# KaffinPX/neptune-core

Measured on AMD Instinct MI355X. Metric: STARK proofs verified/sec (whole node) + Tip5 perms/sec vs VALU roofline, higher is better.
Workload: dtype u64 (Goldilocks mod p; XFE = cubic extension)

## Files before the change

neptune-core_amd/csrc/stark_kernels.hip:

```cpp
#include <hip/hip_ext.h>

#include <atomic>
#include <cstdlib>
#include <type_traits>

#include "../../include/nhip_challenge_id.h"
#include "kernels.hpp"
#include "proof_codec.hpp"
#include "stark.hpp"
#include "stark_launch_plan.hpp"
#include "tip5_device.hpp"
#include "xfe.hpp"

namespace nhip {

#ifndef NHIP_LAT_PRIO
#define NHIP_LAT_PRIO 2
#endif
__device__ __forceinline__ void latency_priority() {
    if constexpr (NHIP_LAT_PRIO > 0) __builtin_amdgcn_s_setprio(NHIP_LAT_PRIO);
}
__device__ uint32_t g_batches_done;
struct AgePrio {
    uint32_t seq, k;
// ... 219 lines not shown
                s[1] = 4 + e < rem ? word_mont<MW>(c1) : (4 + e == rem ? MONT_ONE : 0ull);
                if (r2) s[2] = 8 + e < rem ? word_mont<MW>(c2) : (8 + e == rem ? MONT_ONE : 0ull);
                tip5_permute_quad(s, cq, rck, e, lds.lut);
            }
        } else if (op.kind == FS_SQUEEZE_X) {
            const uint32_t nwords = 3 * op.n;
            for (uint32_t f = 0; f < nwords; f += TIP5_RATE) {
                if (f + e < nwords) xs[xcur + f + e] = s[0];
                if (f + 4 + e < nwords) xs[xcur + f + 4 + e] = s[1];
                if (r2 && f + 8 + e < nwords) xs[xcur + f + 8 + e] = s[2];
                tip5_permute_quad(s, cq, rck, e, lds.lut);
            }
            xcur += nwords;
        } else {
            const uint64_t bound = op.arg;
            uint32_t got = 0;
            while (got < op.n) {
                const uint64_t v0 = from_mont(s[0]), v1 = from_mont(s[1]), v2 = from_mont(s[2]);
                tip5_permute_quad(s, cq, rck, e, lds.lut);
                const bool ok0 = v0 != GL_P - 1, ok1 = v1 != GL_P - 1, ok2 = r2 && v2 != GL_P - 1;
                const uint64_t b0 = __ballot(ok0), b1 = __ballot(ok1), b2 = __ballot(ok2);
                const uint32_t bits = ((uint32_t)(b0 >> qb) & 0xFu) | (((uint32_t)(b1 >> qb) & 0xFu) << 4) |
                                      (((uint32_t)(b2 >> qb) & 0x3u) << 8);
                auto put = [&](bool ok, uint32_t w, uint64_t v) {
                    const uint32_t rank = __popc(bits & ((1u << w) - 1u));
                    if (ok && got + rank < op.n) idx_out[icur + got + rank] = (uint32_t)((v & 0xFFFFFFFFull) % bound);
                };
                put(ok0, e, v0);
                put(ok1, 4 + e, v1);
                put(ok2, 8 + e, v2);
                got += __popc(bits);
            }
            icur += op.n;
        }
    }
}

#ifndef NHIP_ROWS_WAVES
#define NHIP_ROWS_WAVES 5
#endif
#ifndef NHIP_ROWS_WAVES_PLANES
#define NHIP_ROWS_WAVES_PLANES 4
#endif
template <bool MW, bool PLANES>
__global__ void __launch_bounds__(256, PLANES ? NHIP_ROWS_WAVES_PLANES : NHIP_ROWS_WAVES) k_hash_rows(const uint64_t* __restrict__ words, const ProofDesc* __restrict__ desc,
                                                   uint32_t n_proofs, uint32_t k, StarkDims dims,
                                                   uint64_t* __restrict__ dig, const uint32_t* __restrict__ fail,
                                                   AgePrio age) {
    age_priority(age, 0);
    __shared__ Tip5Lds lds;
    tip5_lds_init(lds);
    std::conditional_t<PLANES, Tip5Planes, Tip5NoPlanes> pl;
    if constexpr (PLANES) tip5_planes_init(pl);
    const uint32_t tree = blockIdx.y;
    const uint32_t width = tree == 0 ? dims.num_main : (tree == 1 ? 3 * dims.num_aux : 3 * dims.num_quot_seg);
    for (uint64_t t = blockIdx.x * (uint64_t)blockDim.x + threadIdx.x; t < (uint64_t)n_proofs * k;
         t += (uint64_t)gridDim.x * blockDim.x) {
        const uint32_t p = (uint32_t)(t / k), j = (uint32_t)(t % k);
        if (fail[p]) continue;
        const ProofDesc& d = desc[p];
        const uint64_t base = (tree == 0 ? d.main_rows_off : (tree == 1 ? d.aux_rows_off : d.quot_rows_off)) +
                              (uint64_t)j * width;
        const uint64_t* __restrict__ row = words + base;
        uint64_t s[16];
#pragma unroll
        for (int q = 0; q < 16; ++q) s[q] = 0;
        const uint32_t nchunks = width / TIP5_RATE + 1;
        for (uint32_t c = 0; c < nchunks; ++c) {
            const uint32_t pos = c * TIP5_RATE;
            const bool last = c + 1 == nchunks;
            if (!last) {
#pragma unroll
                for (int q = 0; q < TIP5_RATE; ++q) s[q] = word_mont<MW>(row[pos + q]);
            } else {
                const uint32_t rem = width - pos;
#pragma unroll
                for (int q = 0; q < TIP5_RATE; ++q) {
                    const uint32_t qq = (uint32_t)q;
                    s[q] = qq < rem ? word_mont<MW>(row[pos + qq]) : (qq == rem ? MONT_ONE : 0ull);
                }
            }
            tip5_rounds_0_3(s, lds.lut, pl);
            tip5_last_sbox(s, lds.lut);
            if (!last) tip5_last_mds<10, 16>(s);
            else tip5_last_mds<0, 5>(s);
        }
        uint64_t* __restrict__ o = dig + (((uint64_t)p * 3 + tree) * k + j) * 5;
#pragma unroll
        for (int q = 0; q < 5; ++q) o[q] = s[q];
    }
}

template <bool MW>
__device__ __forceinline__ void hash_rows_wide_body(uint32_t bx, uint32_t tree, const Tip5Lds& t5,
                                                    const uint64_t* __restrict__ words,
                                                    const ProofDesc* __restrict__ desc, uint32_t n_proofs,
                                                    uint32_t k, StarkDims dims, uint64_t* __restrict__ dig,
                                                    const uint32_t* __restrict__ fail) {
    const uint32_t width = tree == 0 ? dims.num_main : (tree == 1 ? 3 * dims.num_aux : 3 * dims.num_quot_seg);
    const uint32_t e = threadIdx.x & 15u;
    const uint64_t t = ((uint64_t)bx * blockDim.x + threadIdx.x) >> 4;
    if (t >= (uint64_t)n_proofs * k) return;
    const uint32_t p = (uint32_t)(t / k), j = (uint32_t)(t % k);
    if (fail[p]) return;
    const ProofDesc& d = desc[p];
    const uint64_t* __restrict__ row =
        words + (tree == 0 ? d.main_rows_off : (tree == 1 ? d.aux_rows_off : d.quot_rows_off)) + (uint64_t)j * width;
    uint64_t rcs[TIP5_ROUNDS];
#pragma unroll
    for (int r = 0; r < TIP5_ROUNDS; ++r) rcs[r] = c_tip5_rc_raw[r * 16 + e];
    const uint32_t nchunks = width / TIP5_RATE + 1;
    auto chunk_word = [&](uint32_t c) -> uint64_t {
        const uint32_t pos = c * TIP5_RATE;
        if (c + 1 < nchunks) return e < TIP5_RATE ? word_mont<MW>(row[pos + e]) : 0ull;
        const uint32_t rem = width - pos;
        return e < rem ? word_mont<MW>(row[pos + e]) : (e == rem ? MONT_ONE : 0ull);
    };
    uint64_t s = 0, next = chunk_word(0);
    for (uint32_t c = 0; c < nchunks; ++c) {
        if (e < TIP5_RATE) s = next;
        if (c + 1 < nchunks) next = chunk_word(c + 1);
        s = tip5_permute_wide<true>(s, e, rcs, t5.lut);
    }
    if (e < 5) dig[(((uint64_t)p * 3 + tree) * k + j) * 5 + e] = s;
}
template <bool MW>
__global__ void __launch_bounds__(256) k_hash_rows_wide(const uint64_t* __restrict__ words,
                                                        const ProofDesc* __restrict__ desc, uint32_t n_proofs,
                                                        uint32_t k, StarkDims dims, uint64_t* __restrict__ dig,
                                                        const uint32_t* __restrict__ fail) {
    latency_priority();
    __shared__ Tip5Lds t5;
    tip5_lds_init(t5);
    hash_rows_wide_body<MW>(blockIdx.x, blockIdx.y, t5, words, desc, n_proofs, k, dims, dig, fail);
}

template <bool MW>
__global__ void __launch_bounds__(256) k_fs_rows_small(const uint64_t* __restrict__ words,
                                                       const ProofDesc* __restrict__ desc,
                                                       const FsOp* __restrict__ ops, uint32_t n_proofs,
                                                       uint64_t* __restrict__ xs, uint32_t* __restrict__ idx_out,
                                                       const uint32_t* __restrict__ fail, AgePrio age,
                                                       uint32_t fs_blocks, uint32_t rows_gx, uint32_t k,
                                                       StarkDims dims, uint64_t* __restrict__ dig) {
    const uint32_t bx = blockIdx.x;
    if (bx < fs_blocks) age_priority(age, NHIP_LAT_PRIO);
    else latency_priority();
    __shared__ Tip5Lds lds;
    tip5_lds_init(lds);
    if (bx < fs_blocks) {
        fs_replay_wide_body<true, MW>(bx, lds, words, desc, ops, n_proofs, xs, idx_out, fail);
    } else {
        const uint32_t r = bx - fs_blocks;
        hash_rows_wide_body<MW>(r % rows_gx, r / rows_gx, lds, words, desc, n_proofs, k, dims, dig, fail);
    }
}

__device__ __forceinline__ void hash_pair_raw(const uint64_t* l, const uint64_t* r, uint64_t* out,
                                              const uint8_t* __restrict__ lut) {
    uint64_t s[16];
#pragma unroll
    for (int q = 0; q < 5; ++q) {
        s[q] = l[q];
        s[5 + q] = r[q];
    }
    tip5_hash_pair_digest(s, lut);
#pragma unroll
// ... 1354 lines not shown
```

neptune-core_amd/csrc/tip5_device.hpp:

```cpp
#pragma once
#include "goldilocks.hpp"
#include "tip5_constants.h"
#include "tip5_mds_planes.hpp"

namespace nhip {

static constexpr int TIP5_STATE = 16;
static constexpr int TIP5_RATE = 10;
static constexpr int TIP5_ROUNDS = 5;
static constexpr uint64_t MONT_ONE = 0x00000000FFFFFFFFull;

__constant__ static uint64_t c_tip5_rc_raw[80] = {
#define NHIP_RC(i) TIP5_RC_RAW[i]
    NHIP_RC(0), NHIP_RC(1), NHIP_RC(2), NHIP_RC(3), NHIP_RC(4), NHIP_RC(5), NHIP_RC(6), NHIP_RC(7),
    NHIP_RC(8), NHIP_RC(9), NHIP_RC(10), NHIP_RC(11), NHIP_RC(12), NHIP_RC(13), NHIP_RC(14), NHIP_RC(15),
    NHIP_RC(16), NHIP_RC(17), NHIP_RC(18), NHIP_RC(19), NHIP_RC(20), NHIP_RC(21), NHIP_RC(22), NHIP_RC(23),
    NHIP_RC(24), NHIP_RC(25), NHIP_RC(26), NHIP_RC(27), NHIP_RC(28), NHIP_RC(29), NHIP_RC(30), NHIP_RC(31),
    NHIP_RC(32), NHIP_RC(33), NHIP_RC(34), NHIP_RC(35), NHIP_RC(36), NHIP_RC(37), NHIP_RC(38), NHIP_RC(39),
    NHIP_RC(40), NHIP_RC(41), NHIP_RC(42), NHIP_RC(43), NHIP_RC(44), NHIP_RC(45), NHIP_RC(46), NHIP_RC(47),
    NHIP_RC(48), NHIP_RC(49), NHIP_RC(50), NHIP_RC(51), NHIP_RC(52), NHIP_RC(53), NHIP_RC(54), NHIP_RC(55),
    NHIP_RC(56), NHIP_RC(57), NHIP_RC(58), NHIP_RC(59), NHIP_RC(60), NHIP_RC(61), NHIP_RC(62), NHIP_RC(63),
    NHIP_RC(64), NHIP_RC(65), NHIP_RC(66), NHIP_RC(67), NHIP_RC(68), NHIP_RC(69), NHIP_RC(70), NHIP_RC(71),
    NHIP_RC(72), NHIP_RC(73), NHIP_RC(74), NHIP_RC(75), NHIP_RC(76), NHIP_RC(77), NHIP_RC(78), NHIP_RC(79),
#undef NHIP_RC
};

__constant__ static uint64_t c_tip5_rck_raw[80] = {
#define NHIP_RC(i) (TIP5_RC_RAW[i] + 0xFFFFFFFFull)
    NHIP_RC(0), NHIP_RC(1), NHIP_RC(2), NHIP_RC(3), NHIP_RC(4), NHIP_RC(5), NHIP_RC(6), NHIP_RC(7),
    NHIP_RC(8), NHIP_RC(9), NHIP_RC(10), NHIP_RC(11), NHIP_RC(12), NHIP_RC(13), NHIP_RC(14), NHIP_RC(15),
    NHIP_RC(16), NHIP_RC(17), NHIP_RC(18), NHIP_RC(19), NHIP_RC(20), NHIP_RC(21), NHIP_RC(22), NHIP_RC(23),
    NHIP_RC(24), NHIP_RC(25), NHIP_RC(26), NHIP_RC(27), NHIP_RC(28), NHIP_RC(29), NHIP_RC(30), NHIP_RC(31),
    NHIP_RC(32), NHIP_RC(33), NHIP_RC(34), NHIP_RC(35), NHIP_RC(36), NHIP_RC(37), NHIP_RC(38), NHIP_RC(39),
    NHIP_RC(40), NHIP_RC(41), NHIP_RC(42), NHIP_RC(43), NHIP_RC(44), NHIP_RC(45), NHIP_RC(46), NHIP_RC(47),
    NHIP_RC(48), NHIP_RC(49), NHIP_RC(50), NHIP_RC(51), NHIP_RC(52), NHIP_RC(53), NHIP_RC(54), NHIP_RC(55),
    NHIP_RC(56), NHIP_RC(57), NHIP_RC(58), NHIP_RC(59), NHIP_RC(60), NHIP_RC(61), NHIP_RC(62), NHIP_RC(63),
    NHIP_RC(64), NHIP_RC(65), NHIP_RC(66), NHIP_RC(67), NHIP_RC(68), NHIP_RC(69), NHIP_RC(70), NHIP_RC(71),
    NHIP_RC(72), NHIP_RC(73), NHIP_RC(74), NHIP_RC(75), NHIP_RC(76), NHIP_RC(77), NHIP_RC(78), NHIP_RC(79),
#undef NHIP_RC
};

struct Tip5Lds {
    uint8_t lut[256];
};

__host__ __device__ constexpr uint32_t tip5_lut_entry(uint32_t x) {
    return ((((x + 1u) * (x + 1u)) % 257u * (x + 1u)) % 257u + 256u) % 257u;
}
constexpr bool tip5_lut_formula_matches_table() {
    for (uint32_t x = 0; x < 256; ++x)
        if (tip5_lut_entry(x) != TIP5_LUT[x]) return false;
    return true;
}
static_assert(tip5_lut_formula_matches_table(), "L(x) = (x+1)^3 - 1 mod 257 is the Tip5 lookup table");

__device__ __forceinline__ void tip5_lds_init(Tip5Lds& lds) {
    for (int i = threadIdx.x; i < 256; i += blockDim.x) lds.lut[i] = TIP5_LUT[i];
    __syncthreads();
}

__device__ __forceinline__ uint32_t lookup4(const uint8_t* __restrict__ lut, uint32_t w) {
    const uint32_t b0 = lut[w & 0xFFu];
    const uint32_t b1 = lut[(w >> 8) & 0xFFu];
    const uint32_t b2 = lut[(w >> 16) & 0xFFu];
    const uint32_t b3 = lut[w >> 24];
    return b0 | (b1 << 8) | (b2 << 16) | (b3 << 24);
}

__device__ __forceinline__ uint64_t split_and_lookup(const uint8_t* __restrict__ lut, uint64_t r) {
    const uint32_t lo = lookup4(lut, (uint32_t)r);
    const uint32_t hi = lookup4(lut, (uint32_t)(r >> 32));
    return ((uint64_t)hi << 32) | lo;
}

__device__ __forceinline__ uint64_t pow7(uint64_t x) {
    const uint64_t x2 = mont_sqr(x);
    const uint64_t x4 = mont_sqr(x2);
    const uint64_t x3 = mont_mul(x, x2);
    return mont_mul(x3, x4);
}

#ifndef NHIP_POW7_GROUP
#define NHIP_POW7_GROUP 3
#endif
__device__ __forceinline__ void mad_carry3(const uint32_t* a1, const uint32_t* b0, const uint64_t* t, uint64_t* u,
                                           uint32_t* c) {
    uint64_t g0, g1, g2;
    asm("v_mad_u64_u32 %0, %6, %9, %12, %15\n\t"
        "v_mad_u64_u32 %1, %7, %10, %13, %16\n\t"
        "v_mad_u64_u32 %2, %8, %11, %14, %17\n\t"
        "v_cndmask_b32_e64 %3, 0, 1, %6\n\t"
        "v_cndmask_b32_e64 %4, 0, 1, %7\n\t"
        "v_cndmask_b32_e64 %5, 0, 1, %8"
        : "=&v"(u[0]), "=&v"(u[1]), "=&v"(u[2]), "=v"(c[0]), "=v"(c[1]), "=v"(c[2]), "=&s"(g0), "=&s"(g1),
          "=&s"(g2)
        : "v"(a1[0]), "v"(a1[1]), "v"(a1[2]), "v"(b0[0]), "v"(b0[1]), "v"(b0[2]), "v"(t[0]), "v"(t[1]), "v"(t[2]));
}

template <int N>
__device__ __forceinline__ void mont_mul_n_dev(const uint64_t* a, const uint64_t* b, uint64_t* out) {
    static_assert(N % 3 == 0, "groups of three");
    uint64_t p00[N], t[N], u[N], xh[N];
    uint32_t a1[N], b0[N], c[N];
    uint32_t ah[N], e[N], bl[N], bh[N], rl[N], rh[N], c1[N], cc[N];
#pragma unroll
    for (int i = 0; i < N; ++i) {
        a1[i] = (uint32_t)(a[i] >> 32);
        b0[i] = (uint32_t)b[i];
        p00[i] = (uint64_t)(uint32_t)a[i] * b0[i];
    }
#pragma unroll
    for (int i = 0; i < N; ++i) t[i] = (uint64_t)(uint32_t)a[i] * (uint32_t)(b[i] >> 32) + (p00[i] >> 32);
#pragma unroll
    for (int i = 0; i < N; i += 3) mad_carry3(a1 + i, b0 + i, t + i, u + i, c + i);
#pragma unroll
    for (int i = 0; i < N; ++i)
        xh[i] = (uint64_t)a1[i] * (uint32_t)(b[i] >> 32) + (((uint64_t)c[i] << 32) | (uint32_t)(u[i] >> 32));
#pragma unroll
    for (int i = 0; i < N; ++i) ah[i] = __builtin_addc((uint32_t)u[i], (uint32_t)p00[i], 0u, &e[i]);
#pragma unroll
    for (int i = 0; i < N; ++i) {
        unsigned int br1;
        bl[i] = __builtin_subc((uint32_t)p00[i], ah[i], e[i], &br1);
        e[i] = br1;
    }
#pragma unroll
    for (int i = 0; i < N; ++i) {
        unsigned int br2;
        bh[i] = __builtin_subc(ah[i], 0u, e[i], &br2);
    }
#pragma unroll
    for (int i = 0; i < N; ++i) rl[i] = __builtin_subc((uint32_t)xh[i], bl[i], 0u, &c1[i]);
#pragma unroll
    for (int i = 0; i < N; ++i) rh[i] = __builtin_subc((uint32_t)(xh[i] >> 32), bh[i], c1[i], &cc[i]);
#pragma unroll
    for (int i = 0; i < N; ++i) {
        unsigned int c2;
        const uint32_t lo = __builtin_subc(rl[i], 0u - cc[i], 0u, &c2);
        out[i] = ((uint64_t)(rh[i] - c2) << 32) | lo;
    }
}

template <int G>
__device__ __forceinline__ void pow7_mul(const uint64_t* a, const uint64_t* b, uint64_t* out) {
    mont_mul_n_dev<G>(a, b, out);
}

__device__ __forceinline__ void pow7_12(uint64_t* x) {
    constexpr int G = NHIP_POW7_GROUP;
    static_assert(12 % G == 0, "group must divide 12");
#pragma unroll
    for (int g = 0; g < 12; g += G) {
        uint64_t x2[G], x4[G], x3[G];
        pow7_mul<G>(x + g, x + g, x2);
        pow7_mul<G>(x2, x2, x4);
        pow7_mul<G>(x + g, x2, x3);
        pow7_mul<G>(x3, x4, x + g);
    }
}

__device__ __forceinline__ void mds_fold4(const uint32_t* sh, const uint64_t* slo, uint64_t* w, uint32_t* e) {
    uint64_t g0, g1, g2, g3;
    asm("v_mad_u64_u32 %0, %8, %12, -1, %16\n\t"
        "v_mad_u64_u32 %1, %9, %13, -1, %17\n\t"
        "v_mad_u64_u32 %2, %10, %14, -1, %18\n\t"
        "v_mad_u64_u32 %3, %11, %15, -1, %19\n\t"
        "v_cndmask_b32_e64 %4, -1, 0, %8\n\t"
        "v_cndmask_b32_e64 %5, -1, 0, %9\n\t"
        "v_cndmask_b32_e64 %6, -1, 0, %10\n\t"
        "v_cndmask_b32_e64 %7, -1, 0, %11"
        : "=&v"(w[0]), "=&v"(w[1]), "=&v"(w[2]), "=&v"(w[3]), "=v"(e[0]), "=v"(e[1]), "=v"(e[2]), "=v"(e[3]),
          "=&s"(g0), "=&s"(g1), "=&s"(g2), "=&s"(g3)
        : "v"(sh[0]), "v"(sh[1]), "v"(sh[2]), "v"(sh[3]), "v"(slo[0]), "v"(slo[1]), "v"(slo[2]), "v"(slo[3]));
}

__device__ __forceinline__ uint64_t mds_reduce_fold(uint64_t al, uint64_t ah);
template <int NIN, int I0, int N>
__device__ __forceinline__ void mds_fold_outputs(const uint32_t* lo, const uint32_t* hi,
                                                 const uint64_t* __restrict__ rck, uint64_t* out) {
    uint64_t al[N], ah[N];
#pragma unroll
    for (int o = 0; o < N; ++o) {
        const int i = I0 + o;
        al[o] = rck[i];
        ah[o] = 0;
#pragma unroll
        for (int j = 0; j < NIN; ++j) {
            const uint64_t c = TIP5_MDS[(i - j) & 15];
            al[o] += c * lo[j];
            ah[o] += c * hi[j];
        }
    }
    constexpr int N4 = N & ~3;
    uint32_t sh[N4 > 0 ? N4 : 1];
    uint64_t slo[N4 > 0 ? N4 : 1], w[N4 > 0 ? N4 : 1];
    uint32_t e[N4 > 0 ? N4 : 1];
#pragma unroll
    for (int o = 0; o < N4; ++o) {
        unsigned int k;
        const uint32_t m1 = __builtin_addc((uint32_t)(al[o] >> 32), (uint32_t)ah[o], 0u, &k);
        sh[o] = (uint32_t)(ah[o] >> 32) + k;
        slo[o] = ((uint64_t)m1 << 32) | (uint32_t)al[o];
    }
#pragma unroll
    for (int o = 0; o < N4; o += 4) mds_fold4(sh + o, slo + o, w + o, e + o);
#pragma unroll
    for (int o = 0; o < N4; ++o) out[o] = w[o] - e[o];
#pragma unroll
    for (int o = N4; o < N; ++o) out[o] = mds_reduce_fold(al[o], ah[o]);
}

#ifndef NHIP_PAIR_MDS_GROUP
#define NHIP_PAIR_MDS_GROUP 2
#endif
#ifndef NHIP_SPONGE_MDS_GROUP
#define NHIP_SPONGE_MDS_GROUP 4
#endif
template <int NIN, int OBEG, int OEND, int G>
__device__ __forceinline__ void mds_fold_groups(const uint32_t* lo, const uint32_t* hi,
                                                const uint64_t* __restrict__ rck, uint64_t* out) {
    constexpr int N = (OEND - OBEG) < G ? (OEND - OBEG) : G;
    mds_fold_outputs<NIN, OBEG, N>(lo, hi, rck, out);
    if constexpr (OBEG + N < OEND) {
        __builtin_amdgcn_sched_barrier(0);
        mds_fold_groups<NIN, OBEG + N, OEND, G>(lo, hi, rck, out + N);
    }
}

template <int NIN, int OBEG = 0, int OEND = 16, int G = 16>
__device__ __forceinline__ void mds_ark_fold(uint64_t s[16], const uint64_t* __restrict__ rck) {
    uint32_t lo[NIN], hi[NIN];
#pragma unroll
    for (int j = 0; j < NIN; ++j) {
        lo[j] = (uint32_t)s[j];
        hi[j] = (uint32_t)(s[j] >> 32);
    }
    uint64_t out[OEND - OBEG];
    mds_fold_groups<NIN, OBEG, OEND, G>(lo, hi, rck, out);
#pragma unroll
    for (int o = 0; o < OEND - OBEG; ++o) s[OBEG + o] = out[o];
}

template <int G = NHIP_SPONGE_MDS_GROUP>
__device__ __forceinline__ void mds_ark(uint64_t s[16], const uint64_t* __restrict__ rc,
                                        const uint64_t* __restrict__ rck) {
    (void)rc;
    mds_ark_fold<16, 0, 16, G>(s, rck);
}

typedef int tip5_v4i __attribute__((ext_vector_type(4)));
typedef int tip5_v16i __attribute__((ext_vector_type(16)));

struct Tip5PlanesTable {
    uint32_t w[3 * 64 * 4];
};
constexpr Tip5PlanesTable tip5_planes_table() {
    Tip5PlanesTable tb{};
    for (int e = 0; e < 3; ++e)
        for (int l = 0; l < 64; ++l)
            for (int t = 0; t < 16; ++t)
                tb.w[(e * 64 + l) * 4 + t / 4] |= (uint32_t)(uint8_t)(int8_t)planes_tile_byte(e, l, t) << (8 * (t % 4));
    return tb;
}
__constant__ static Tip5PlanesTable c_tip5_planes_tiles = tip5_planes_table();

__constant__ static uint64_t c_tip5_rckp_raw[80] = {
#define NHIP_RC(i) planes_start(TIP5_RC_RAW[i] + 0xFFFFFFFFull)
    NHIP_RC(0), NHIP_RC(1), NHIP_RC(2), NHIP_RC(3), NHIP_RC(4), NHIP_RC(5), NHIP_RC(6), NHIP_RC(7),
    NHIP_RC(8), NHIP_RC(9), NHIP_RC(10), NHIP_RC(11), NHIP_RC(12), NHIP_RC(13), NHIP_RC(14), NHIP_RC(15),
    NHIP_RC(16), NHIP_RC(17), NHIP_RC(18), NHIP_RC(19), NHIP_RC(20), NHIP_RC(21), NHIP_RC(22), NHIP_RC(23),
    NHIP_RC(24), NHIP_RC(25), NHIP_RC(26), NHIP_RC(27), NHIP_RC(28), NHIP_RC(29), NHIP_RC(30), NHIP_RC(31),
    NHIP_RC(32), NHIP_RC(33), NHIP_RC(34), NHIP_RC(35), NHIP_RC(36), NHIP_RC(37), NHIP_RC(38), NHIP_RC(39),
    NHIP_RC(40), NHIP_RC(41), NHIP_RC(42), NHIP_RC(43), NHIP_RC(44), NHIP_RC(45), NHIP_RC(46), NHIP_RC(47),
    NHIP_RC(48), NHIP_RC(49), NHIP_RC(50), NHIP_RC(51), NHIP_RC(52), NHIP_RC(53), NHIP_RC(54), NHIP_RC(55),
    NHIP_RC(56), NHIP_RC(57), NHIP_RC(58), NHIP_RC(59), NHIP_RC(60), NHIP_RC(61), NHIP_RC(62), NHIP_RC(63),
    NHIP_RC(64), NHIP_RC(65), NHIP_RC(66), NHIP_RC(67), NHIP_RC(68), NHIP_RC(69), NHIP_RC(70), NHIP_RC(71),
    NHIP_RC(72), NHIP_RC(73), NHIP_RC(74), NHIP_RC(75), NHIP_RC(76), NHIP_RC(77), NHIP_RC(78), NHIP_RC(79),
#undef NHIP_RC
};

struct Tip5Planes {
    tip5_v4i tile[3];
    int32_t k0, k8, k16, k24;
};
__device__ __forceinline__ void tip5_planes_init(Tip5Planes& pl) {
    const uint32_t lane = __builtin_amdgcn_mbcnt_hi(~0u, __builtin_amdgcn_mbcnt_lo(~0u, 0u));
    const tip5_v4i* tb = (const tip5_v4i*)c_tip5_planes_tiles.w;
#pragma unroll
    for (int e = 0; e < 3; ++e) {
        pl.tile[e] = tb[e * 64 + lane];
        asm volatile("" : "+v"(pl.tile[e]));
    }
    asm("v_mov_b32 %0, 1" : "=v"(pl.k0));
    asm("s_mov_b32 %0, 0x100" : "=s"(pl.k8));
    asm("s_mov_b32 %0, 0x10000" : "=s"(pl.k16));
    asm("s_mov_b32 %0, 0x1000000" : "=s"(pl.k24));
}

template <int Q>
__device__ __forceinline__ tip5_v16i planes_cq(const Tip5Planes& pl, const tip5_v4i* plane) {
    tip5_v16i c = {0, 0, 0, 0, 0, 0, 0, 0, 0, 0, 0, 0, 0, 0, 0, 0};
#pragma unroll
    for (int e = 0; e < 3; ++e)
        if (Q - e >= 0 && Q - e <= 7) c = __builtin_amdgcn_mfma_i32_32x32x32_i8(pl.tile[e], plane[Q - e], c, 0, 0, 0);
    return c;
}

__device__ __forceinline__ int64_t planes_mad(int32_t c, int32_t k, int64_t a) { return (int64_t)c * (int64_t)k + a; }

__host__ __device__ constexpr int planes_order(int k) {
    constexpr int o[10] = {0, 1, 2, 3, 9, 8, 4, 5, 6, 7};
    return o[k];
}
template <int K>
__device__ __forceinline__ void planes_step(const Tip5Planes& pl, const tip5_v4i* plane, const tip5_v16i& c,
                                            const uint64_t* __restrict__ rckp, int64_t* al, int64_t* t, uint32_t* hb) {
    constexpr int Q = planes_order(K);
    tip5_v16i next;
    if constexpr (K < 9) next = planes_cq<planes_order(K + 1)>(pl, plane);
#pragma unroll
    for (int i = 0; i < 16; ++i) {
        if constexpr (Q == 0) al[i] = planes_mad(c[i], pl.k0, (int64_t)rckp[i]);
        if constexpr (Q == 1) al[i] = planes_mad(c[i], pl.k8, al[i]);
        if constexpr (Q == 2) al[i] = planes_mad(c[i], pl.k16, al[i]);
        if constexpr (Q == 3) al[i] = planes_mad(c[i], pl.k24, al[i]);
        if constexpr (Q == 9) hb[i] = ((uint32_t)c[i] << 8) + (uint32_t)PLANES_HB_BIAS;
        if constexpr (Q == 8) t[i] = (int64_t)(((uint64_t)(hb[i] + (uint32_t)c[i]) << 32) | (uint32_t)((uint64_t)al[i] >> 32));
        if constexpr (Q == 4) t[i] = planes_mad(c[i], pl.k0, t[i]);
        if constexpr (Q == 5) t[i] = planes_mad(c[i], pl.k8, t[i]);
        if constexpr (Q == 6) t[i] = planes_mad(c[i], pl.k16, t[i]);
        if constexpr (Q == 7) t[i] = planes_mad(c[i], pl.k24, t[i]);
    }
    if constexpr (K < 9) {
        __builtin_amdgcn_sched_barrier(0);
        planes_step<K + 1>(pl, plane, next, rckp, al, t, hb);
    }
}

__device__ __forceinline__ void mds_ark_planes(uint64_t s[16], const uint64_t* __restrict__ rckp, const Tip5Planes& pl) {
    tip5_v4i plane[8];
#pragma unroll
    for (int m = 0; m < 4; ++m)
#pragma unroll
        for (int h = 0; h < 2; ++h) {
            uint32_t w[4];
#pragma unroll
            for (int b = 0; b < 4; ++b) w[b] = (uint32_t)(s[4 * m + b] >> (32 * h)) ^ 0x80808080u;
            const uint32_t a0 = __builtin_amdgcn_perm(w[1], w[0], 0x05010400u);
            const uint32_t a1 = __builtin_amdgcn_perm(w[1], w[0], 0x07030602u);
            const uint32_t c0 = __builtin_amdgcn_perm(w[3], w[2], 0x05010400u);
            const uint32_t c1 = __builtin_amdgcn_perm(w[3], w[2], 0x07030602u);
            plane[4 * h + 0][m] = (int)__builtin_amdgcn_perm(c0, a0, 0x05040100u);
            plane[4 * h + 1][m] = (int)__builtin_amdgcn_perm(c0, a0, 0x07060302u);
            plane[4 * h + 2][m] = (int)__builtin_amdgcn_perm(c1, a1, 0x05040100u);
            plane[4 * h + 3][m] = (int)__builtin_amdgcn_perm(c1, a1, 0x07060302u);
        }
    int64_t al[16], t[16];
    uint32_t hb[16];
    planes_step<0>(pl, plane, planes_cq<0>(pl, plane), rckp, al, t, hb);
    uint32_t sh[16], e[16];
    uint64_t slo[16], w[16];
#pragma unroll
    for (int i = 0; i < 16; ++i) {
        sh[i] = (uint32_t)((uint64_t)t[i] >> 32);
        slo[i] = ((uint64_t)t[i] << 32) | (uint32_t)al[i];
    }
#pragma unroll
    for (int i = 0; i < 16; i += 4) mds_fold4(sh + i, slo + i, w + i, e + i);
#pragma unroll
    for (int i = 0; i < 16; ++i) s[i] = w[i] - e[i];
}

struct Tip5NoPlanes {};
template <class PL>
inline constexpr bool tip5_is_planes = false;
template <>
inline constexpr bool tip5_is_planes<Tip5Planes> = true;
template <int G, class PL>
__device__ __forceinline__ void mds_ark_round(uint64_t s[16], int r, const PL& pl) {
    if constexpr (tip5_is_planes<PL>) mds_ark_planes(s, c_tip5_rckp_raw + r * 16, pl);
    else mds_ark<G>(s, c_tip5_rc_raw + r * 16, c_tip5_rck_raw + r * 16);
}

template <class PL = Tip5NoPlanes>
__device__ __forceinline__ void tip5_permute_raw(uint64_t s[16], const uint8_t* __restrict__ lut, const PL& pl = PL{}) {
#pragma unroll 1
    for (int r = 0; r < TIP5_ROUNDS; ++r) {
#pragma unroll
        for (int i = 0; i < 4; ++i) s[i] = split_and_lookup(lut, s[i]);
        pow7_12(s + 4);
        mds_ark_round<NHIP_SPONGE_MDS_GROUP>(s, r, pl);
    }
}


__host__ __device__ constexpr uint64_t tip5_rck0_fixed(int i) {
    uint64_t k = TIP5_RC_RAW[i] + 0xFFFFFFFFull;
    for (int j = 10; j < 16; ++j) k += (uint64_t)TIP5_MDS[(i - j) & 15] * 0xFFFFFFFFull;
    return k;
}
constexpr bool tip5_rck0_fixed_in_range() {
    for (int i = 0; i < 16; ++i)
        if (tip5_rck0_fixed(i) >= 0xFFF0000000000000ull || tip5_rck0_fixed(i) < TIP5_RC_RAW[i]) return false;
    return true;
}
static_assert(tip5_rck0_fixed_in_range(), "round-0 FixedLength accumulator start below 2^64 - 2^52");
__constant__ static uint64_t c_tip5_rck0_fixed[16] = {
    tip5_rck0_fixed(0),  tip5_rck0_fixed(1),  tip5_rck0_fixed(2),  tip5_rck0_fixed(3),
    tip5_rck0_fixed(4),  tip5_rck0_fixed(5),  tip5_rck0_fixed(6),  tip5_rck0_fixed(7),
    tip5_rck0_fixed(8),  tip5_rck0_fixed(9),  tip5_rck0_fixed(10), tip5_rck0_fixed(11),
    tip5_rck0_fixed(12), tip5_rck0_fixed(13), tip5_rck0_fixed(14), tip5_rck0_fixed(15),
};

template <class PL = Tip5NoPlanes>
__device__ __forceinline__ void tip5_hash_pair_digest(uint64_t s[16], const uint8_t* __restrict__ lut, const PL& pl = PL{}) {
#pragma unroll
    for (int i = 0; i < 4; ++i) s[i] = split_and_lookup(lut, s[i]);
#pragma unroll
    for (int g = 4; g < 10; g += 3) {
        uint64_t x2[3], x4[3], x3[3];
        pow7_mul<3>(s + g, s + g, x2);
        pow7_mul<3>(x2, x2, x4);
        pow7_mul<3>(s + g, x2, x3);
        pow7_mul<3>(x3, x4, s + g);
    }
    mds_ark_fold<10, 0, 16, NHIP_PAIR_MDS_GROUP>(s, c_tip5_rck0_fixed);
#pragma unroll 1
    for (int r = 1; r < TIP5_ROUNDS - 1; ++r) {
#pragma unroll
        for (int i = 0; i < 4; ++i) s[i] = split_and_lookup(lut, s[i]);
        pow7_12(s + 4);
        mds_ark_round<NHIP_PAIR_MDS_GROUP>(s, r, pl);
    }
#pragma unroll
    for (int i = 0; i < 4; ++i) s[i] = split_and_lookup(lut, s[i]);
    pow7_12(s + 4);
    mds_ark_fold<16, 0, 5, NHIP_PAIR_MDS_GROUP>(s, c_tip5_rck_raw + (TIP5_ROUNDS - 1) * 16);
}

template <class PL = Tip5NoPlanes>
__device__ __forceinline__ void tip5_rounds_0_3(uint64_t s[16], const uint8_t* __restrict__ lut, const PL& pl = PL{}) {
#pragma unroll 1
    for (int r = 0; r < TIP5_ROUNDS - 1; ++r) {
#pragma unroll
        for (int i = 0; i < 4; ++i) s[i] = split_and_lookup(lut, s[i]);
        pow7_12(s + 4);
        mds_ark_round<NHIP_SPONGE_MDS_GROUP>(s, r, pl);
    }
}
__device__ __forceinline__ void tip5_last_sbox(uint64_t s[16], const uint8_t* __restrict__ lut) {
#pragma unroll
    for (int i = 0; i < 4; ++i) s[i] = split_and_lookup(lut, s[i]);
    pow7_12(s + 4);
}
template <int OBEG, int OEND>
__device__ __forceinline__ void tip5_last_mds(uint64_t s[16]) {
    mds_ark_fold<16, OBEG, OEND, NHIP_SPONGE_MDS_GROUP>(s, c_tip5_rck_raw + (TIP5_ROUNDS - 1) * 16);
}
template <int OBEG, int OEND>
__device__ __forceinline__ void tip5_last_round(uint64_t s[16], const uint8_t* __restrict__ lut) {
    tip5_last_sbox(s, lut);
    tip5_last_mds<OBEG, OEND>(s);
}

}

namespace nhip {

__device__ __forceinline__ uint64_t mds_reduce_ark_lat(uint64_t al, uint64_t ah, uint64_t nq) {
    const uint64_t w = (uint64_t)(uint32_t)(al >> 32) + (uint32_t)ah;
    const uint32_t sh = (uint32_t)(ah >> 32) + (uint32_t)(w >> 32);
    const uint64_t slo = ((uint64_t)(uint32_t)w << 32) | (uint32_t)al;
    const uint64_t res = slo + (uint64_t)sh * 0xFFFFFFFFull;
    const uint64_t y = res + (res < slo ? GL_EPS : 0ull);
    const uint64_t x1 = y + nq;
    return x1 + (x1 > y ? GL_P : 0ull);
}

__device__ __forceinline__ uint64_t mds_reduce_fold(uint64_t al, uint64_t ah) {
    unsigned int k;
    const uint32_t m1 = __builtin_addc((uint32_t)(al >> 32), (uint32_t)ah, 0u, &k);
    const uint32_t sh = (uint32_t)(ah >> 32) + k;
    const uint64_t slo = ((uint64_t)m1 << 32) | (uint32_t)al;
    uint64_t w, g;
    uint32_t e;
    asm("v_mad_u64_u32 %0, %2, %3, -1, %4\n\t"
        "s_nop 1\n\t"
        "v_cndmask_b32_e64 %1, -1, 0, %2"
        : "=&v"(w), "=v"(e), "=&s"(g)
        : "v"(sh), "v"(slo));
    return w - e;
}

template <bool LAT>
__device__ __forceinline__ uint64_t mont_mul_sel(uint64_t a, uint64_t b) {
    if constexpr (LAT) return mont_mul_lat(a, b);
    else return mont_mul(a, b);
}

template <int K>
__device__ __forceinline__ uint32_t row_ror(uint32_t v) {
    return (uint32_t)__builtin_amdgcn_mov_dpp((int)v, 0x120 + K, 0xF, 0xF, false);
}

template <int K>
__device__ __forceinline__ void mds_term(uint32_t lo, uint32_t hi, uint64_t& al, uint64_t& ah) {
    const uint64_t c = TIP5_MDS[K];
    al += c * row_ror<K>(lo);
    ah += c * row_ror<K>(hi);
}

template <bool LAT>
__device__ __forceinline__ uint64_t tip5_permute_wide(uint64_t s, uint32_t e, const uint64_t rc[5],
                                                      const uint8_t* __restrict__ lut) {
#pragma unroll
    for (int r = 0; r < TIP5_ROUNDS; ++r) {
        {
            const uint64_t lk = split_and_lookup(lut, s);
            const uint64_t x2 = mont_mul_sel<LAT>(s, s);
            const uint64_t x4 = mont_mul_sel<LAT>(x2, x2);
            const uint64_t x3 = mont_mul_sel<LAT>(s, x2);
            const uint64_t x7 = mont_mul_sel<LAT>(x3, x4);
            s = e < 4 ? lk : x7;
        }
        const uint32_t lo = (uint32_t)s, hi = (uint32_t)(s >> 32);
        uint64_t al, ah;
        if constexpr (LAT) {
            al = (uint64_t)TIP5_MDS[0] * lo;
            ah = (uint64_t)TIP5_MDS[0] * hi;
        } else {
            al = (uint64_t)TIP5_MDS[0] * lo + (rc[r] + GL_EPS);
            ah = (uint64_t)TIP5_MDS[0] * hi;
        }
        mds_term<1>(lo, hi, al, ah);
        mds_term<2>(lo, hi, al, ah);
        mds_term<3>(lo, hi, al, ah);
        mds_term<4>(lo, hi, al, ah);
        mds_term<5>(lo, hi, al, ah);
        mds_term<6>(lo, hi, al, ah);
        mds_term<7>(lo, hi, al, ah);
        mds_term<8>(lo, hi, al, ah);
        mds_term<9>(lo, hi, al, ah);
        mds_term<10>(lo, hi, al, ah);
        mds_term<11>(lo, hi, al, ah);
        mds_term<12>(lo, hi, al, ah);
        mds_term<13>(lo, hi, al, ah);
        mds_term<14>(lo, hi, al, ah);
        mds_term<15>(lo, hi, al, ah);
        if constexpr (LAT) s = mds_reduce_ark_lat(al, ah, 0ull - (GL_P - rc[r]));
        else s = mds_reduce_fold(al, ah);
    }
    return s;
}

__device__ __forceinline__ void row_pair(uint64_t x, uint64_t& r0, uint64_t& r1) {
    const auto lo = __builtin_amdgcn_permlane16_swap((uint32_t)x, (uint32_t)x, false, false);
    const auto hi = __builtin_amdgcn_permlane16_swap((uint32_t)(x >> 32), (uint32_t)(x >> 32), false, false);
    r0 = ((uint64_t)hi[0] << 32) | lo[0];
    r1 = ((uint64_t)hi[1] << 32) | lo[1];
}

template <int K>
__device__ __forceinline__ void mds_term_pair(uint32_t lo, uint32_t hi, uint32_t c, uint64_t& al, uint64_t& ah) {
    al += (uint64_t)c * row_ror<K>(lo);
    ah += (uint64_t)c * row_ror<K>(hi);
}

__device__ __forceinline__ uint64_t tip5_permute_pair(uint64_t s, uint32_t e, uint32_t h, const uint64_t rc[5],
                                                      const uint32_t cm[8], const uint8_t* __restrict__ lut) {
#pragma unroll
    for (int r = 0; r < TIP5_ROUNDS; ++r) {
        const uint32_t lk_mine = lookup4(lut, h ? (uint32_t)(s >> 32) : (uint32_t)s);
        const uint64_t x2 = mont_mul_lat(s, s);
        const uint64_t m = mont_mul_lat(h ? s : x2, x2);
// ... 101 lines not shown
```

Before: 504,300.

## Keep non-canonical Tip5 words feeding x^7 and fold lookup XOR into LUT

```diff
diff --git a/neptune-core_amd/csrc/stark_kernels.hip b/neptune-core_amd/csrc/stark_kernels.hip
--- a/neptune-core_amd/csrc/stark_kernels.hip
+++ b/neptune-core_amd/csrc/stark_kernels.hip
@@ -325,7 +325,7 @@
             }
             tip5_rounds_0_3(s, lds.lut, pl);
             tip5_last_sbox(s, lds.lut);
-            if (!last) tip5_last_mds<10, 16>(s);
+            if (!last) tip5_last_mds<10, 16, true>(s);
             else tip5_last_mds<0, 5>(s);
         }
         uint64_t* __restrict__ o = dig + (((uint64_t)p * 3 + tree) * k + j) * 5;
diff --git a/neptune-core_amd/csrc/tip5_device.hpp b/neptune-core_amd/csrc/tip5_device.hpp
--- a/neptune-core_amd/csrc/tip5_device.hpp
+++ b/neptune-core_amd/csrc/tip5_device.hpp
@@ -40,9 +40,37 @@
 #undef NHIP_RC
 };
 
+__host__ __device__ constexpr bool tip5_word_any(int i) { return i >= 4; }
+__host__ __device__ constexpr uint64_t tip5_rca(int i) {
+    return TIP5_RC_RAW[i] + ((i < 64 && tip5_word_any(i & 15)) ? 0ull : 0xFFFFFFFFull);
+}
+constexpr bool tip5_rc_starts_in_range() {
+    for (int i = 0; i < 80; ++i)
+        if (TIP5_RC_RAW[i] >= 0ull - (1ull << 52) || tip5_rca(i) >= 0ull - (1ull << 52)) return false;
+    return true;
+}
+static_assert(tip5_rc_starts_in_range(), "rc + 2^52 does not overflow for any Tip5 round constant");
+__constant__ static uint64_t c_tip5_rca_raw[80] = {
+#define NHIP_RC(i) tip5_rca(i)
+    NHIP_RC(0), NHIP_RC(1), NHIP_RC(2), NHIP_RC(3), NHIP_RC(4), NHIP_RC(5), NHIP_RC(6), NHIP_RC(7),
+    NHIP_RC(8), NHIP_RC(9), NHIP_RC(10), NHIP_RC(11), NHIP_RC(12), NHIP_RC(13), NHIP_RC(14), NHIP_RC(15),
+    NHIP_RC(16), NHIP_RC(17), NHIP_RC(18), NHIP_RC(19), NHIP_RC(20), NHIP_RC(21), NHIP_RC(22), NHIP_RC(23),
+    NHIP_RC(24), NHIP_RC(25), NHIP_RC(26), NHIP_RC(27), NHIP_RC(28), NHIP_RC(29), NHIP_RC(30), NHIP_RC(31),
+    NHIP_RC(32), NHIP_RC(33), NHIP_RC(34), NHIP_RC(35), NHIP_RC(36), NHIP_RC(37), NHIP_RC(38), NHIP_RC(39),
+    NHIP_RC(40), NHIP_RC(41), NHIP_RC(42), NHIP_RC(43), NHIP_RC(44), NHIP_RC(45), NHIP_RC(46), NHIP_RC(47),
+    NHIP_RC(48), NHIP_RC(49), NHIP_RC(50), NHIP_RC(51), NHIP_RC(52), NHIP_RC(53), NHIP_RC(54), NHIP_RC(55),
+    NHIP_RC(56), NHIP_RC(57), NHIP_RC(58), NHIP_RC(59), NHIP_RC(60), NHIP_RC(61), NHIP_RC(62), NHIP_RC(63),
+    NHIP_RC(64), NHIP_RC(65), NHIP_RC(66), NHIP_RC(67), NHIP_RC(68), NHIP_RC(69), NHIP_RC(70), NHIP_RC(71),
+    NHIP_RC(72), NHIP_RC(73), NHIP_RC(74), NHIP_RC(75), NHIP_RC(76), NHIP_RC(77), NHIP_RC(78), NHIP_RC(79),
+#undef NHIP_RC
+};
+
 struct Tip5Lds {
     uint8_t lut[256];
-};
+    uint8_t lutx[256];
+};
+static constexpr int TIP5_LUTX = 256;
+static_assert(offsetof(Tip5Lds, lutx) == offsetof(Tip5Lds, lut) + TIP5_LUTX, "lutx follows lut");
 
 __host__ __device__ constexpr uint32_t tip5_lut_entry(uint32_t x) {
     return ((((x + 1u) * (x + 1u)) % 257u * (x + 1u)) % 257u + 256u) % 257u;
@@ -55,7 +83,12 @@
 static_assert(tip5_lut_formula_matches_table(), "L(x) = (x+1)^3 - 1 mod 257 is the Tip5 lookup table");
 
 __device__ __forceinline__ void tip5_lds_init(Tip5Lds& lds) {
-    for (int i = threadIdx.x; i < 256; i += blockDim.x) lds.lut[i] = TIP5_LUT[i];
+#pragma unroll 1
+    for (int i = threadIdx.x; i < 256; i += blockDim.x) {
+        const uint8_t v = TIP5_LUT[i];
+        lds.lut[i] = v;
+        lds.lutx[i] = v ^ 0x80u;
+    }
     __syncthreads();
 }
 
@@ -174,8 +207,39 @@
         : "v"(sh[0]), "v"(sh[1]), "v"(sh[2]), "v"(sh[3]), "v"(slo[0]), "v"(slo[1]), "v"(slo[2]), "v"(slo[3]));
 }
 
+__device__ __forceinline__ void mds_fold4_any(const uint32_t* sh, const uint64_t* slo, uint64_t* out) {
+    uint64_t g[4], b[4], w[4];
+    uint32_t lo[4], hi[4];
+    asm("v_mad_u64_u32 %0, %4, %8, -1, %12\n\t"
+        "v_mad_u64_u32 %1, %5, %9, -1, %13\n\t"
+        "v_mad_u64_u32 %2, %6, %10, -1, %14\n\t"
+        "v_mad_u64_u32 %3, %7, %11, -1, %15"
+        : "=&v"(w[0]), "=&v"(w[1]), "=&v"(w[2]), "=&v"(w[3]), "=&s"(g[0]), "=&s"(g[1]), "=&s"(g[2]), "=&s"(g[3])
+        : "v"(sh[0]), "v"(sh[1]), "v"(sh[2]), "v"(sh[3]), "v"(slo[0]), "v"(slo[1]), "v"(slo[2]), "v"(slo[3]));
+    asm("v_subb_co_u32_e64 %0, %8, %12, 0, %20\n\t"
+        "v_subb_co_u32_e64 %1, %9, %13, 0, %21\n\t"
+        "v_subb_co_u32_e64 %2, %10, %14, 0, %22\n\t"
+        "v_subb_co_u32_e64 %3, %11, %15, 0, %23\n\t"
+        "s_andn2_b64 %8, %20, %8\n\t"
+        "s_andn2_b64 %9, %21, %9\n\t"
+        "s_andn2_b64 %10, %22, %10\n\t"
+        "s_andn2_b64 %11, %23, %11\n\t"
+        "v_addc_co_u32_e64 %4, %8, %16, 0, %8\n\t"
+        "v_addc_co_u32_e64 %5, %9, %17, 0, %9\n\t"
+        "v_addc_co_u32_e64 %6, %10, %18, 0, %10\n\t"
+        "v_addc_co_u32_e64 %7, %11, %19, 0, %11"
+        : "=&v"(lo[0]), "=&v"(lo[1]), "=&v"(lo[2]), "=&v"(lo[3]), "=&v"(hi[0]), "=&v"(hi[1]), "=&v"(hi[2]),
+          "=&v"(hi[3]), "=&s"(b[0]), "=&s"(b[1]), "=&s"(b[2]), "=&s"(b[3])
+        : "v"((uint32_t)w[0]), "v"((uint32_t)w[1]), "v"((uint32_t)w[2]), "v"((uint32_t)w[3]),
+          "v"((uint32_t)(w[0] >> 32)), "v"((uint32_t)(w[1] >> 32)), "v"((uint32_t)(w[2] >> 32)),
+          "v"((uint32_t)(w[3] >> 32)), "s"(g[0]), "s"(g[1]), "s"(g[2]), "s"(g[3])
+        : "scc");
+#pragma unroll
+    for (int q = 0; q < 4; ++q) out[q] = ((uint64_t)hi[q] << 32) | lo[q];
+}
 __device__ __forceinline__ uint64_t mds_reduce_fold(uint64_t al, uint64_t ah);
-template <int NIN, int I0, int N>
+__device__ __forceinline__ uint64_t mds_reduce_fold_any(uint64_t al, uint64_t ah);
+template <int NIN, int I0, int N, bool ANY = false>
 __device__ __forceinline__ void mds_fold_outputs(const uint32_t* lo, const uint32_t* hi,
                                                  const uint64_t* __restrict__ rck, uint64_t* out) {
     uint64_t al[N], ah[N];
@@ -203,11 +267,24 @@
         slo[o] = ((uint64_t)m1 << 32) | (uint32_t)al[o];
     }
 #pragma unroll
-    for (int o = 0; o < N4; o += 4) mds_fold4(sh + o, slo + o, w + o, e + o);
-#pragma unroll
-    for (int o = 0; o < N4; ++o) out[o] = w[o] - e[o];
-#pragma unroll
-    for (int o = N4; o < N; ++o) out[o] = mds_reduce_fold(al[o], ah[o]);
+    for (int o = 0; o < N4; o += 4) {
+        if (ANY && tip5_word_any(I0 + o)) {
+            mds_fold4_any(sh + o, slo + o, out + o);
+        } else {
+            mds_fold4(sh + o, slo + o, w + o, e + o);
+#pragma unroll
+            for (int q = o; q < o + 4; ++q) out[q] = w[q] - e[q];
+        }
+    }
+#pragma unroll
+    for (int o = N4; o < N; ++o)
+        out[o] = (ANY && tip5_word_any(I0 + o)) ? mds_reduce_fold_any(al[o], ah[o]) : mds_reduce_fold(al[o], ah[o]);
+}
+template <int I0, int N>
+constexpr bool mds_fold_blocks_unmixed() {
+    for (int o = 0; o + 4 <= N; o += 4)
+        if (tip5_word_any(I0 + o) != tip5_word_any(I0 + o + 3)) return false;
+    return true;
 }
 
 #ifndef NHIP_PAIR_MDS_GROUP
@@ -216,18 +293,19 @@
 #ifndef NHIP_SPONGE_MDS_GROUP
 #define NHIP_SPONGE_MDS_GROUP 4
 #endif
-template <int NIN, int OBEG, int OEND, int G>
+template <int NIN, int OBEG, int OEND, int G, bool ANY = false>
 __device__ __forceinline__ void mds_fold_groups(const uint32_t* lo, const uint32_t* hi,
                                                 const uint64_t* __restrict__ rck, uint64_t* out) {
     constexpr int N = (OEND - OBEG) < G ? (OEND - OBEG) : G;
-    mds_fold_outputs<NIN, OBEG, N>(lo, hi, rck, out);
+    static_assert(!ANY || mds_fold_blocks_unmixed<OBEG, N>(), "a block of four is canonical or any as a whole");
+    mds_fold_outputs<NIN, OBEG, N, ANY>(lo, hi, rck, out);
     if constexpr (OBEG + N < OEND) {
         __builtin_amdgcn_sched_barrier(0);
-        mds_fold_groups<NIN, OBEG + N, OEND, G>(lo, hi, rck, out + N);
-    }
-}
-
-template <int NIN, int OBEG = 0, int OEND = 16, int G = 16>
+        mds_fold_groups<NIN, OBEG + N, OEND, G, ANY>(lo, hi, rck, out + N);
+    }
+}
+
+template <int NIN, int OBEG = 0, int OEND = 16, int G = 16, bool ANY = false>
 __device__ __forceinline__ void mds_ark_fold(uint64_t s[16], const uint64_t* __restrict__ rck) {
     uint32_t lo[NIN], hi[NIN];
 #pragma unroll
@@ -236,7 +314,7 @@
         hi[j] = (uint32_t)(s[j] >> 32);
     }
     uint64_t out[OEND - OBEG];
-    mds_fold_groups<NIN, OBEG, OEND, G>(lo, hi, rck, out);
+    mds_fold_groups<NIN, OBEG, OEND, G, ANY>(lo, hi, rck, out);
 #pragma unroll
     for (int o = 0; o < OEND - OBEG; ++o) s[OBEG + o] = out[o];
 }
@@ -279,6 +357,27 @@
 #undef NHIP_RC
 };
 
+constexpr bool planes_any_starts_in_range() {
+    for (int i = 0; i < 80; ++i)
+        if (!planes_start_in_range(TIP5_RC_RAW[i])) return false;
+    return true;
+}
+static_assert(planes_any_starts_in_range(), "planes_start(RC) in [2^45, 2^64 - 2^45) for every Tip5 round constant");
+__constant__ static uint64_t c_tip5_rcap_raw[80] = {
+#define NHIP_RC(i) planes_start(tip5_rca(i))
+    NHIP_RC(0), NHIP_RC(1), NHIP_RC(2), NHIP_RC(3), NHIP_RC(4), NHIP_RC(5), NHIP_RC(6), NHIP_RC(7),
+    NHIP_RC(8), NHIP_RC(9), NHIP_RC(10), NHIP_RC(11), NHIP_RC(12), NHIP_RC(13), NHIP_RC(14), NHIP_RC(15),
+    NHIP_RC(16), NHIP_RC(17), NHIP_RC(18), NHIP_RC(19), NHIP_RC(20), NHIP_RC(21), NHIP_RC(22), NHIP_RC(23),
+    NHIP_RC(24), NHIP_RC(25), NHIP_RC(26), NHIP_RC(27), NHIP_RC(28), NHIP_RC(29), NHIP_RC(30), NHIP_RC(31),
+    NHIP_RC(32), NHIP_RC(33), NHIP_RC(34), NHIP_RC(35), NHIP_RC(36), NHIP_RC(37), NHIP_RC(38), NHIP_RC(39),
+    NHIP_RC(40), NHIP_RC(41), NHIP_RC(42), NHIP_RC(43), NHIP_RC(44), NHIP_RC(45), NHIP_RC(46), NHIP_RC(47),
+    NHIP_RC(48), NHIP_RC(49), NHIP_RC(50), NHIP_RC(51), NHIP_RC(52), NHIP_RC(53), NHIP_RC(54), NHIP_RC(55),
+    NHIP_RC(56), NHIP_RC(57), NHIP_RC(58), NHIP_RC(59), NHIP_RC(60), NHIP_RC(61), NHIP_RC(62), NHIP_RC(63),
+    NHIP_RC(64), NHIP_RC(65), NHIP_RC(66), NHIP_RC(67), NHIP_RC(68), NHIP_RC(69), NHIP_RC(70), NHIP_RC(71),
+    NHIP_RC(72), NHIP_RC(73), NHIP_RC(74), NHIP_RC(75), NHIP_RC(76), NHIP_RC(77), NHIP_RC(78), NHIP_RC(79),
+#undef NHIP_RC
+};
+
 struct Tip5Planes {
     tip5_v4i tile[3];
     int32_t k0, k8, k16, k24;
@@ -337,6 +436,7 @@
     }
 }
 
+template <bool ANY = false, bool PRE = false>
 __device__ __forceinline__ void mds_ark_planes(uint64_t s[16], const uint64_t* __restrict__ rckp, const Tip5Planes& pl) {
     tip5_v4i plane[8];
 #pragma unroll
@@ -345,7 +445,7 @@
         for (int h = 0; h < 2; ++h) {
             uint32_t w[4];
 #pragma unroll
-            for (int b = 0; b < 4; ++b) w[b] = (uint32_t)(s[4 * m + b] >> (32 * h)) ^ 0x80808080u;
+            for (int b = 0; b < 4; ++b) w[b] = (uint32_t)(s[4 * m + b] >> (32 * h)) ^ ((PRE && m == 0) ? 0u : 0x80808080u);
             const uint32_t a0 = __builtin_amdgcn_perm(w[1], w[0], 0x05010400u);
             const uint32_t a1 = __builtin_amdgcn_perm(w[1], w[0], 0x07030602u);
             const uint32_t c0 = __builtin_amdgcn_perm(w[3], w[2], 0x05010400u);
@@ -366,9 +466,16 @@
         slo[i] = ((uint64_t)t[i] << 32) | (uint32_t)al[i];
     }
 #pragma unroll
-    for (int i = 0; i < 16; i += 4) mds_fold4(sh + i, slo + i, w + i, e + i);
-#pragma unroll
-    for (int i = 0; i < 16; ++i) s[i] = w[i] - e[i];
+    for (int i = 0; i < 16; i += 4) {
+        static_assert(!tip5_word_any(3) && tip5_word_any(4), "blocks of four are canonical or any as a whole");
+        if (ANY && tip5_word_any(i)) {
+            mds_fold4_any(sh + i, slo + i, s + i);
+        } else {
+            mds_fold4(sh + i, slo + i, w + i, e + i);
+#pragma unroll
+            for (int q = i; q < i + 4; ++q) s[q] = w[q] - e[q];
+        }
+    }
 }
 
 struct Tip5NoPlanes {};
@@ -376,21 +483,26 @@
 inline constexpr bool tip5_is_planes = false;
 template <>
 inline constexpr bool tip5_is_planes<Tip5Planes> = true;
+template <int G, bool ANY, class PL>
+__device__ __forceinline__ void tip5_full_round(uint64_t s[16], int r, const uint8_t* __restrict__ lut, const PL& pl) {
+    constexpr bool P = tip5_is_planes<PL>;
+#pragma unroll
+    for (int i = 0; i < 4; ++i) s[i] = split_and_lookup(P ? lut + TIP5_LUTX : lut, s[i]);
+    pow7_12(s + 4);
+    if constexpr (P) mds_ark_planes<ANY, true>(s, (ANY ? c_tip5_rcap_raw : c_tip5_rckp_raw) + r * 16, pl);
+    else mds_ark_fold<16, 0, 16, G, ANY>(s, (ANY ? c_tip5_rca_raw : c_tip5_rck_raw) + r * 16);
+}
+
 template <int G, class PL>
-__device__ __forceinline__ void mds_ark_round(uint64_t s[16], int r, const PL& pl) {
-    if constexpr (tip5_is_planes<PL>) mds_ark_planes(s, c_tip5_rckp_raw + r * 16, pl);
-    else mds_ark<G>(s, c_tip5_rc_raw + r * 16, c_tip5_rck_raw + r * 16);
+__device__ __forceinline__ void tip5_rounds_0_3_g(uint64_t s[16], const uint8_t* __restrict__ lut, const PL& pl) {
+#pragma unroll 1
+    for (int r = 0; r < TIP5_ROUNDS - 1; ++r) tip5_full_round<G, true>(s, r, lut, pl);
 }
 
 template <class PL = Tip5NoPlanes>
 __device__ __forceinline__ void tip5_permute_raw(uint64_t s[16], const uint8_t* __restrict__ lut, const PL& pl = PL{}) {
-#pragma unroll 1
-    for (int r = 0; r < TIP5_ROUNDS; ++r) {
-#pragma unroll
-        for (int i = 0; i < 4; ++i) s[i] = split_and_lookup(lut, s[i]);
-        pow7_12(s + 4);
-        mds_ark_round<NHIP_SPONGE_MDS_GROUP>(s, r, pl);
-    }
+    tip5_rounds_0_3_g<NHIP_SPONGE_MDS_GROUP>(s, lut, pl);
+    tip5_full_round<NHIP_SPONGE_MDS_GROUP, false>(s, TIP5_ROUNDS - 1, lut, pl);
 }
 
 
@@ -411,6 +523,21 @@
     tip5_rck0_fixed(8),  tip5_rck0_fixed(9),  tip5_rck0_fixed(10), tip5_rck0_fixed(11),
     tip5_rck0_fixed(12), tip5_rck0_fixed(13), tip5_rck0_fixed(14), tip5_rck0_fixed(15),
 };
+__host__ __device__ constexpr uint64_t tip5_rca0_fixed(int i) {
+    return tip5_rck0_fixed(i) - (tip5_word_any(i) ? 0xFFFFFFFFull : 0ull);
+}
+constexpr bool tip5_rca0_fixed_in_range() {
+    for (int i = 0; i < 16; ++i)
+        if (tip5_rca0_fixed(i) >= 0xFFF0000000000000ull || tip5_rca0_fixed(i) < TIP5_RC_RAW[i]) return false;
+    return true;
+}
+static_assert(tip5_rca0_fixed_in_range(), "round-0 FixedLength any-representative start below 2^64 - 2^52");
+__constant__ static uint64_t c_tip5_rca0_fixed[16] = {
+    tip5_rca0_fixed(0),  tip5_rca0_fixed(1),  tip5_rca0_fixed(2),  tip5_rca0_fixed(3),
+    tip5_rca0_fixed(4),  tip5_rca0_fixed(5),  tip5_rca0_fixed(6),  tip5_rca0_fixed(7),
+    tip5_rca0_fixed(8),  tip5_rca0_fixed(9),  tip5_rca0_fixed(10), tip5_rca0_fixed(11),
+    tip5_rca0_fixed(12), tip5_rca0_fixed(13), tip5_rca0_fixed(14), tip5_rca0_fixed(15),
+};
 
 template <class PL = Tip5NoPlanes>
 __device__ __forceinline__ void tip5_hash_pair_digest(uint64_t s[16], const uint8_t* __restrict__ lut, const PL& pl = PL{}) {
@@ -424,14 +551,9 @@
         pow7_mul<3>(s + g, x2, x3);
         pow7_mul<3>(x3, x4, s + g);
     }
-    mds_ark_fold<10, 0, 16, NHIP_PAIR_MDS_GROUP>(s, c_tip5_rck0_fixed);
+    mds_ark_fold<10, 0, 16, NHIP_PAIR_MDS_GROUP, true>(s, c_tip5_rca0_fixed);
 #pragma unroll 1
-    for (int r = 1; r < TIP5_ROUNDS - 1; ++r) {
-#pragma unroll
-        for (int i = 0; i < 4; ++i) s[i] = split_and_lookup(lut, s[i]);
-        pow7_12(s + 4);
-        mds_ark_round<NHIP_PAIR_MDS_GROUP>(s, r, pl);
-    }
+    for (int r = 1; r < TIP5_ROUNDS - 1; ++r) tip5_full_round<NHIP_PAIR_MDS_GROUP, true>(s, r, lut, pl);
 #pragma unroll
     for (int i = 0; i < 4; ++i) s[i] = split_and_lookup(lut, s[i]);
     pow7_12(s + 4);
@@ -440,22 +562,17 @@
 
 template <class PL = Tip5NoPlanes>
 __device__ __forceinline__ void tip5_rounds_0_3(uint64_t s[16], const uint8_t* __restrict__ lut, const PL& pl = PL{}) {
-#pragma unroll 1
-    for (int r = 0; r < TIP5_ROUNDS - 1; ++r) {
-#pragma unroll
-        for (int i = 0; i < 4; ++i) s[i] = split_and_lookup(lut, s[i]);
-        pow7_12(s + 4);
-        mds_ark_round<NHIP_SPONGE_MDS_GROUP>(s, r, pl);
-    }
+    tip5_rounds_0_3_g<NHIP_SPONGE_MDS_GROUP>(s, lut, pl);
 }
 __device__ __forceinline__ void tip5_last_sbox(uint64_t s[16], const uint8_t* __restrict__ lut) {
 #pragma unroll
     for (int i = 0; i < 4; ++i) s[i] = split_and_lookup(lut, s[i]);
     pow7_12(s + 4);
 }
-template <int OBEG, int OEND>
+template <int OBEG, int OEND, bool ANY = false>
 __device__ __forceinline__ void tip5_last_mds(uint64_t s[16]) {
-    mds_ark_fold<16, OBEG, OEND, NHIP_SPONGE_MDS_GROUP>(s, c_tip5_rck_raw + (TIP5_ROUNDS - 1) * 16);
+    static_assert(!ANY || tip5_word_any(OBEG), "every kept word feeds x^7");
+    mds_ark_fold<16, OBEG, OEND, NHIP_SPONGE_MDS_GROUP, ANY>(s, (ANY ? c_tip5_rc_raw : c_tip5_rck_raw) + (TIP5_ROUNDS - 1) * 16);
 }
 template <int OBEG, int OEND>
 __device__ __forceinline__ void tip5_last_round(uint64_t s[16], const uint8_t* __restrict__ lut) {
@@ -490,6 +607,23 @@
         : "=&v"(w), "=v"(e), "=&s"(g)
         : "v"(sh), "v"(slo));
     return w - e;
+}
+__device__ __forceinline__ uint64_t mds_reduce_fold_any(uint64_t al, uint64_t ah) {
+    unsigned int k;
+    const uint32_t m1 = __builtin_addc((uint32_t)(al >> 32), (uint32_t)ah, 0u, &k);
+    const uint32_t sh = (uint32_t)(ah >> 32) + k;
+    const uint64_t slo = ((uint64_t)m1 << 32) | (uint32_t)al;
+    uint64_t w, g, b;
+    uint32_t lo, hi;
+    asm("v_mad_u64_u32 %0, %1, %2, -1, %3" : "=&v"(w), "=&s"(g) : "v"(sh), "v"(slo));
+    asm("s_nop 1\n\t"
+        "v_subb_co_u32_e64 %0, %2, %3, 0, %5\n\t"
+        "s_andn2_b64 %2, %5, %2\n\t"
+        "v_addc_co_u32_e64 %1, %2, %4, 0, %2"
+        : "=&v"(lo), "=&v"(hi), "=&s"(b)
+        : "v"((uint32_t)w), "v"((uint32_t)(w >> 32)), "s"(g)
+        : "scc");
+    return ((uint64_t)hi << 32) | lo;
 }
 
 template <bool LAT>
```

Result: no change. 500,700 (-0.7%).
